# facebook/zstd

Hardware: NVIDIA H100
Metric: compress GB/s (input) at level 1 (higher is better)
Workload: dtype u8

## Files before the change

zstd_b200/csrc/zb_entropy.cuh:

```cuda
#ifndef ZB_ENTROPY_CUH
#define ZB_ENTROPY_CUH
#include "zb_device.cuh"

#define ZBD_ERR 0xFFFFFFFFu

struct ZbdBitW { u8* out; u32 pos; u64 acc; u32 nacc; };
__device__ __forceinline__ void zbd_bw_init(ZbdBitW* w, u8* out) { w->out = out; w->pos = 0; w->acc = 0; w->nacc = 0; }
__device__ __forceinline__ void zbd_bw_add(ZbdBitW* w, u32 value, u32 nbBits)
{
    if (!nbBits) return;
    w->acc |= (u64)(value & ((1u << nbBits) - 1u)) << w->nacc;
    w->nacc += nbBits;
    while (w->nacc >= 8) { w->out[w->pos++] = (u8)w->acc; w->acc >>= 8; w->nacc -= 8; }
}
__device__ __forceinline__ u32 zbd_bw_close(ZbdBitW* w)
{
    zbd_bw_add(w, 1, 1);
    if (w->nacc) w->out[w->pos++] = (u8)w->acc;
    return w->pos;
}


__device__ __forceinline__ u32 zbd_fse_optimalTableLog(u32 maxTableLog, u32 srcSize, u32 maxSymbolValue, u32 minus)
{
    u32 const fromSource = zb_hb32(srcSize - 1u) - minus;
    u32 const needSrc = zb_hb32(srcSize) + 1u, needAlphabet = zb_hb32(maxSymbolValue) + 2u;
    u32 const floorLog = needSrc < needAlphabet ? needSrc : needAlphabet;
    u32 log = maxTableLog < fromSource ? maxTableLog : fromSource;
    if (log < floorLog) log = floorLog;
    return log < 5u ? 5u : (log > 12u ? 12u : log);
}

__device__ inline u32 zbw_fse_normalize(short* norm, u32 tableLog, const u32* count, u32 total, u32 maxSymbolValue, u32 lane)
{
    u32 const T = 1u << tableLog;
    u32 base[2], rem[2]; bool present[2];
#pragma unroll
// ... 128 lines not shown
            u32 const owner = ls >> 1;
            u32 const before = __shfl_sync(ZB_FULL, (ls & 1u) ? seen1 : seen0, (int)owner);
            if (s == ls) ct->nextState[cum[ls] + before + (u32)__popc(grp & ((1u << lane) - 1u))] = (u16)(T + u);
            if (lane == owner) { if (ls & 1u) seen1 += (u32)__popc(grp); else seen0 += (u32)__popc(grp); }
            pending &= ~grp;
        }
    }
    __syncwarp();
}

__device__ inline void zbd_fse_buildCTable_rle(ZbdFseCTable* ct, u32 symbol)
{
    ct->tableLog = 0; ct->maxSymbolValue = symbol;
    ct->nextState[0] = 0; ct->nextState[1] = 0;
    ct->deltaNbBits[symbol] = 0; ct->deltaFindState[symbol] = 0;
}

__device__ __forceinline__ u32 zbd_fse_initState2(const ZbdFseCTable* ct, u32 symbol)
{
    u32 const dnb = ct->deltaNbBits[symbol];
    u32 const nbBitsOut = (dnb + (1u << 15)) >> 16;
    u32 const value = (nbBitsOut << 16) - dnb;
    return ct->nextState[(int)(value >> nbBitsOut) + ct->deltaFindState[symbol]];
}
__device__ __forceinline__ u32 zbd_fse_step(const ZbdFseCTable* ct, u32 state, u32 symbol, u32* bits, u32* nb)
{
    u32 const nbBitsOut = (state + ct->deltaNbBits[symbol]) >> 16;
    *nb = nbBitsOut;
    *bits = state & ((1u << nbBitsOut) - 1u);
    return ct->nextState[(int)(state >> nbBitsOut) + ct->deltaFindState[symbol]];
}

struct ZbdHufWksp {
    u32 A[256];
    u16 rankSym[256];
    u8  len[256];
    u8  weights[256];
    u32 nl[16];
    u32 firstCode[16];
    u32 wcount[16];
    short wnorm[16];
    u8  symAt[64];
    u16 cum[66];
    u32 maxLen, nz;
    ZbdFseCTable wct;
};

template <int HUF_THREADS>
__device__ inline u32 zbc_huf_build(ZbdHufWksp* w, const u32* count, u32 maxSymbolValue, u32 target, u32* enc)
{
    u32 const tid = threadIdx.x;
    if (tid == 0) w->nz = 0;
    __syncthreads();
    {   u32 mine = 0;
        for (u32 s = tid; s < 256u; s += HUF_THREADS) {
            u32 const c = s <= maxSymbolValue ? count[s] : 0u;
            w->len[s] = 0;
            if (c) {
                u32 r = 0;
                for (u32 j = 0; j <= maxSymbolValue; j++) { u32 const cj = count[j]; r += (cj > c || (cj == c && j < s)) ? 1u : 0u; }
                w->rankSym[r] = (u16)s;
                mine++;
            }
        }
        if (mine) atomicAdd(&w->nz, mine);
    }
    __syncthreads();
    u32 const nz = w->nz;
    for (u32 i = tid; i < nz; i += HUF_THREADS) w->A[i] = count[w->rankSym[nz - 1u - i]];
    __syncthreads();
    if (tid == 0) {
        u32* const A = w->A;
        u32 root = 0, leaf = 2, next;
        A[0] += A[1];
        for (next = 1; next + 1u < nz; next++) {
            if (leaf >= nz || A[root] < A[leaf]) { A[next] = A[root]; A[root++] = next; } else A[next] = A[leaf++];
            if (leaf >= nz || (root < next && A[root] < A[leaf])) { A[next] += A[root]; A[root++] = next; } else A[next] += A[leaf++];
        }
        A[nz - 2u] = 0;
        for (next = nz - 2u; next-- > 0u; ) A[next] = A[A[next]] + 1u;
        {   int avbl = 1, used = 0, depth = 0;
            int rt = (int)nz - 2, nx = (int)nz - 1;
            while (avbl > 0) {
                while (rt >= 0 && (int)A[rt] == depth) { used++; rt--; }
                while (avbl > used) { A[nx--] = (u32)depth; avbl--; }
                avbl = 2 * used; depth++; used = 0;
            }
        }
        for (u32 l = 0; l < 16u; l++) w->nl[l] = 0;
    }
    __syncthreads();
    u32 const deepest = w->A[0];
    for (u32 i = tid; i < nz; i += HUF_THREADS) { u32 const l = w->A[i]; atomicAdd(&w->nl[l < 15u ? l : 15u], 1u); }
    __syncthreads();
    if (tid == 0) {
        u32* const nl = w->nl;
        u32 maxLen = deepest;
        if (maxLen > target) {
            u32 K = 0;
            for (u32 l = target + 1u; l < 16u; l++) { nl[target] += nl[l]; nl[l] = 0; }
            for (u32 l = 1; l <= target; l++) K += nl[l] << (target - l);
            for (u32 E = K - (1u << target); E > 0u; E--) {
                u32 b = target - 1u;
                while (nl[b] == 0u) b--;
                nl[b]--; nl[b + 1u] += 2u; nl[target]--;
            }
            maxLen = target;
        }
        while (nl[maxLen] == 0u) maxLen--;
        w->maxLen = maxLen;
        u32 v = 0;
        for (u32 l = maxLen; l > 0u; l--) { w->firstCode[l] = v; v = (v + nl[l]) >> 1; }
    }
    __syncthreads();
    u32 const maxLen = w->maxLen;
    for (u32 r = tid; r < nz; r += HUF_THREADS) {
        u32 l = 1, acc = w->nl[1];
        while (r >= acc) { l++; acc += w->nl[l]; }
        w->len[w->rankSym[r]] = (u8)l;
    }
    __syncthreads();
    for (u32 s = tid; s < 256u; s += HUF_THREADS) {
        u32 const l = w->len[s];
        u32 e = 0;
        if (l) {
            u32 idx = 0;
            for (u32 j = 0; j < s; j++) idx += (w->len[j] == l) ? 1u : 0u;
            e = (w->firstCode[l] + idx) | (l << 16);
        }
        enc[s] = e;
    }
    __syncthreads();
    return maxLen;
}

template <int HUF_THREADS>
__device__ inline u32 zbc_huf_writeHeader(ZbdHufWksp* w, u8* dst, const u32* enc, u32 maxSymbolValue, u32 huffLog, u32* sh_result)
{
    u32 const tid = threadIdx.x, lane = tid & 31u;
    u8* const wt = w->weights;
    u32 const wtSize = maxSymbolValue;
    if (tid < 16u) w->wcount[tid] = 0;
    __syncthreads();
    for (u32 n = tid; n < wtSize; n += HUF_THREADS) {
        u32 const nb = enc[n] >> 16;
        u32 const v = nb ? huffLog + 1u - nb : 0u;
        wt[n] = (u8)v;
        atomicAdd(&w->wcount[v], 1u);
    }
    if (tid == 0) wt[wtSize] = 0;
    __syncthreads();
    if (tid < 32u) {
        u32 hSize = 0;
        if (wtSize > 2u) {
            u32 const c = lane < 13u ? w->wcount[lane] : 0u;
            u32 const used = __ballot_sync(ZB_FULL, c != 0u);
            u32 const maxSym = 31u - (u32)__clz((int)used);
            u32 maxCount = c;
#pragma unroll
            for (u32 o = 16; o > 0; o >>= 1) maxCount = max(maxCount, __shfl_xor_sync(ZB_FULL, maxCount, o));
            if (maxCount != wtSize && maxCount != 1u) {
                u32 const tableLog = zbd_fse_optimalTableLog(6, wtSize, maxSym, 2);
                u32 ok = zbw_fse_normalize(w->wnorm, tableLog, w->wcount, wtSize, maxSym, lane);
                u32 nc = 0;
                if (ok != ZBD_ERR) {
                    if (lane == 0) nc = zbd_fse_writeNCount(dst + 1, w->wnorm, maxSym, tableLog);
                    nc = __shfl_sync(ZB_FULL, nc, 0);
                    if (nc == ZBD_ERR) ok = ZBD_ERR;
                }
                if (ok != ZBD_ERR) {
                    zbw_fse_buildCTable(&w->wct, w->wnorm, maxSym, tableLog, w->symAt, w->cum, lane);
                    if (lane == 0) {
                        ZbdBitW bw; zbd_bw_init(&bw, dst + 1 + nc);
                        const u8* ip = wt + wtSize;
                        u32 s1, s2, bits, nb;
                        if (wtSize & 1u) {
                            s1 = zbd_fse_initState2(&w->wct, *--ip);
                            s2 = zbd_fse_initState2(&w->wct, *--ip);
                            s1 = zbd_fse_step(&w->wct, s1, *--ip, &bits, &nb); zbd_bw_add(&bw, bits, nb);
                        } else {
                            s2 = zbd_fse_initState2(&w->wct, *--ip);
                            s1 = zbd_fse_initState2(&w->wct, *--ip);
                        }
                        while (ip > wt) {
                            s2 = zbd_fse_step(&w->wct, s2, *--ip, &bits, &nb); zbd_bw_add(&bw, bits, nb);
                            s1 = zbd_fse_step(&w->wct, s1, *--ip, &bits, &nb); zbd_bw_add(&bw, bits, nb);
                        }
                        zbd_bw_add(&bw, s2, tableLog);
                        zbd_bw_add(&bw, s1, tableLog);
                        hSize = nc + zbd_bw_close(&bw);
                    }
                } else if (lane == 0) hSize = ZBD_ERR;
            } else if (maxCount == wtSize) hSize = 1;
        }
        if (lane == 0) {
            u32 res;
            if (hSize == ZBD_ERR) res = ZBD_ERR;
            else if (hSize > 1u && hSize < maxSymbolValue / 2u) { dst[0] = (u8)hSize; res = hSize + 1u; }
            else if (maxSymbolValue > 128u) res = ZBD_ERR;
            else {
                dst[0] = (u8)(128u + (maxSymbolValue - 1u));
                for (u32 n = 0; n < maxSymbolValue; n += 2u) dst[(n / 2u) + 1u] = (u8)((wt[n] << 4) + wt[n + 1u]);
                res = ((maxSymbolValue + 1u) / 2u) + 1u;
            }
            *sh_result = res;
        }
    }
    __syncthreads();
    return *sh_result;
}
#endif
```

zstd_b200/csrc/zb_literals.cu:

```cuda
#include "zb_entropy.cuh"
#include "zb_kernels.h"

#define LIT_THREADS 128
#ifndef LIT_MIN_CTAS
#define LIT_MIN_CTAS 12
#endif
#define LIT_WARPS (LIT_THREADS / 32)
#define LIT_WIN 256u

__device__ void zb_hist256(const u8* __restrict__ src, u32 n, u32 (*whist)[256], u32* count)
{
    u32 const tid = threadIdx.x, warp = tid >> 5, lane = tid & 31u;
    for (u32 i = tid; i < LIT_WARPS * 256; i += LIT_THREADS) (&whist[0][0])[i] = 0;
    __syncthreads();
    u32 const head = (u32)((uintptr_t)src & 15u);
    const uint4* const v4 = reinterpret_cast<const uint4*>(src - head);
    u32 const seg = (n + 3u) / 4u;
    u32 const beg = min(warp * seg, n) + head, end = min((warp + 1u) * seg, n) + head;
    if (beg < end) {
        u32 const vLo = beg >> 4, nVec = ((end - 1u) >> 4) - vLo + 1u;
        uint4 nx = lane < nVec ? __ldg(v4 + vLo + lane) : make_uint4(0, 0, 0, 0);
        for (u32 i = lane; i < nVec; i += 32u) {
            uint4 const q = nx;
            if (i + 32u < nVec) nx = __ldg(v4 + vLo + i + 32u);
            u32 const p0 = (vLo + i) << 4;
            u32 const kLo = beg > p0 ? beg - p0 : 0u, kHi = min(end - p0, 16u);
            u32 const w[4] = { q.x, q.y, q.z, q.w };
#pragma unroll
            for (u32 k = 0; k < 16u; k++)
                if (k >= kLo && k < kHi) atomicAdd(&whist[warp][(w[k >> 2] >> (8u * (k & 3u))) & 0xFFu], 1u);
        }
    }
    __syncthreads();
    for (u32 sym = tid; sym < 256u; sym += LIT_THREADS) {
        u32 s = 0;
#pragma unroll
        for (int w = 0; w < LIT_WARPS; w++) s += whist[w][sym];
        count[sym] = s;
    }
    __syncthreads();
}

__device__ void zb_hist_stats(const u32* count, u32* red, u32* largestOut, u32* maxSymOut)
{
    u32 const tid = threadIdx.x;
    u32 c = 0, key = 0;
    for (u32 sym = tid; sym < 256u; sym += LIT_THREADS) { u32 const v = count[sym]; c = max(c, v); key = max(key, v ? sym : 0u); }
#pragma unroll
    for (int o = 16; o > 0; o >>= 1) {
        c = max(c, __shfl_xor_sync(ZB_FULL, c, o));
        key = max(key, __shfl_xor_sync(ZB_FULL, key, o));
    }
    if ((tid & 31) == 0) { red[tid >> 5] = c; red[8 + (tid >> 5)] = key; }
    __syncthreads();
    if (tid == 0) {
        u32 l = 0, m = 0;
        for (int w = 0; w < LIT_WARPS; w++) { l = max(l, red[w]); m = max(m, red[8 + w]); }
        *largestOut = l; *maxSymOut = m;
    }
    __syncthreads();
}

__device__ __forceinline__ void zb_huf_stream(const u8* __restrict__ lit, u32 beg, u32 end, const u32* enc, u32* win, u32* ow,
                                              u32 bitPos, u32 lane)
{
    const uint4* const v4 = reinterpret_cast<const uint4*>(lit);
    uint4 const zero = make_uint4(0, 0, 0, 0);
    u32 const vHi = (end - 1u) >> 4, nVec = vHi - (beg >> 4) + 1u;
    u32 const firstW = bitPos >> 5;
    uint4 q1 = lane < nVec ? __ldg(v4 + vHi - lane) : zero;
    uint4 q2 = lane + 32u < nVec ? __ldg(v4 + vHi - lane - 32u) : zero;
    for (u32 t = 0; t < nVec; t += 32u) {
        uint4 const q = q1;
        q1 = q2;
        q2 = t + 64u + lane < nVec ? __ldg(v4 + vHi - (t + 64u + lane)) : zero;
        u32 kLo = 0, kHi = 0;
        if (t + lane < nVec) { u32 const p0 = (vHi - t - lane) << 4; kLo = beg > p0 ? beg - p0 : 0u; kHi = min(end - p0, 16u); }
        u32 const w[4] = { q.x, q.y, q.z, q.w };
        u32 nb = 0;
#pragma unroll
        for (u32 k = 0; k < 16u; k++) {
            u32 const e = enc[(w[k >> 2] >> (8u * (k & 3u))) & 0xFFu];
            nb += (k >= kLo && k < kHi) ? e >> 16 : 0u;
        }
        u32 incl = nb;
#pragma unroll
        for (u32 o = 1; o < 32u; o <<= 1) { u32 const x = __shfl_up_sync(ZB_FULL, incl, o); if (lane >= o) incl += x; }
        u32 const tileBits = __shfl_sync(ZB_FULL, incl, 31);
        {
            u32 const p = bitPos + incl - nb;
            u32 widx = p >> 5, nacc = p & 31u, first = 1;
            u64 acc = 0;
#pragma unroll
            for (int k = 15; k >= 0; k--) {
                u32 const e = ((u32)k >= kLo && (u32)k < kHi) ? enc[(w[k >> 2] >> (8u * (k & 3u))) & 0xFFu] : 0u;
                acc |= (u64)(e & 0xFFFFu) << nacc;
                nacc += e >> 16;
                if (k & 1) continue;
                bool const full = nacc >= 32u;
                u32* const wp = win + widx % LIT_WIN;
                if (full && first == 0u) *wp = (u32)acc;
                if (full && first != 0u) atomicOr(wp, (u32)acc);
                first = full ? 0u : first;
                widx += full ? 1u : 0u;
                acc = full ? (acc >> 32) : acc;
                nacc -= full ? 32u : 0u;
            }
            if (nacc != 0u && (u32)acc != 0u) atomicOr(win + widx % LIT_WIN, (u32)acc);
        }
        __syncwarp();
        u32 const wEnd = (bitPos + tileBits) >> 5;
        for (u32 k = (bitPos >> 5) + lane; k < wEnd; k += 32u) {
            u32 const v = win[k % LIT_WIN];
            win[k % LIT_WIN] = 0u;
            if (k == firstW) atomicOr(ow + k, v); else ow[k] = v;
        }
        __syncwarp();
        bitPos += tileBits;
    }
    if (lane == 0) atomicOr(ow + (bitPos >> 5), win[(bitPos >> 5) % LIT_WIN] | (1u << (bitPos & 31u)));
}

__global__ void __launch_bounds__(LIT_THREADS, LIT_MIN_CTAS)
zb_literals_kernel(const ZbBlock* __restrict__ blocks, ZbParams prm, ZbStrides sd, const ZbDictEntropy* __restrict__ deAll,
                   const ZbDictSlot* __restrict__ dicts, const u8* __restrict__ lits, u8* __restrict__ body, ZbBlockMeta* __restrict__ meta)
{
    __shared__ __align__(16) u32 whist[LIT_WARPS][256];
    __shared__ ZbdHufWksp wk;
    __shared__ u32 count[256];
    __shared__ u32 enc[256];
    __shared__ __align__(16) u8 hdr[288];
    __shared__ u32 red[16];
    __shared__ u32 sh_largest, sh_maxSym, sh_mode, sh_hSize, sh_usePrev;
    __shared__ u32 sh_bits[LIT_WARPS];

    u32 const tid = threadIdx.x, warp = tid >> 5, lane = tid & 31u;
    u32 const b = blockIdx.x;
    ZbBlockMeta const m = meta[b];
    if (m.forceRaw) return;
    u32 const n = m.litSize;
    const u8* const lit = lits + (size_t)b * sd.lit;
    u8* const out = body + (size_t)b * sd.body;
    enum { MODE_RAW = 0, MODE_RLE = 1, MODE_HUF = 2 };

    ZbBlock const bd = blocks[b];
    const ZbDictEntropy* const de = (bd.flags & ZB_FLAG_FIRST) ? (dicts ? dicts[bd.dictSlot].de : deAll) : nullptr;
    u32 repeat = (de != nullptr && de->present) ? de->hufRepeat : 0u;
    bool const preferRepeat = (n <= 1024u);
    u32 const lhSize = 3u + (n >= 1024u) + (n >= 16384u);
    u32 const nbStreams = (n < 256u || (repeat == 2u && lhSize == 3u)) ? 1u : 4u;
    u32 mode = MODE_HUF;
    bool usePrev = false;
    if (prm.litDisabled || n < (repeat == 2u ? 6u : 64u)) mode = MODE_RAW;
    if (mode == MODE_HUF && preferRepeat && repeat == 2u) usePrev = true;
    if (mode == MODE_HUF && !usePrev) {
        bool const suspect = (m.nbSeq == 0) || (n / m.nbSeq >= 20u);
        if (suspect && n >= 4096u * 10u) {
            u32 l1, l2;
            zb_hist256(lit, 4096u, whist, count);
            zb_hist_stats(count, red, &sh_largest, &sh_maxSym);
            l1 = sh_largest;
            __syncthreads();
            zb_hist256(lit + n - 4096u, 4096u, whist, count);
            zb_hist_stats(count, red, &sh_largest, &sh_maxSym);
            l2 = sh_largest;
            __syncthreads();
            if (l1 + l2 <= ((2u * 4096u) >> 7) + 4u) mode = MODE_RAW;
        }
    }
    if (mode == MODE_HUF) zb_hist256(lit, n, whist, count);
    if (mode == MODE_HUF && !usePrev) {
        zb_hist_stats(count, red, &sh_largest, &sh_maxSym);
        u32 const largest = sh_largest;
        if (largest == n) mode = MODE_RLE;
        else if (largest <= (n >> 7) + 4u) mode = MODE_RAW;
    }
    if (mode == MODE_HUF && !usePrev && repeat == 1u) {
        int bad = 0;
        for (u32 sym = tid; sym < 256u; sym += LIT_THREADS) bad |= (sym <= sh_maxSym) && count[sym] != 0u && (de->hufEnc[sym] >> 16) == 0u;
        if (__syncthreads_or(bad) || de->hufMaxSymbol < sh_maxSym) repeat = 0u;
    }
    if (mode == MODE_HUF && !usePrev && preferRepeat && repeat != 0u) usePrev = true;
    if (mode == MODE_HUF && !usePrev) {
        u32 const maxSym = sh_maxSym;
        u32 const huffLog = zbd_fse_optimalTableLog(11, n, maxSym, 1);
        u32 const maxBits = zbc_huf_build<LIT_THREADS>(&wk, count, maxSym, huffLog, enc);
        u32 const hSizeNew = (maxBits == ZBD_ERR) ? ZBD_ERR : zbc_huf_writeHeader<LIT_THREADS>(&wk, hdr, enc, maxSym, maxBits, &sh_hSize);
        if (tid == 0) {
            u32 md = MODE_HUF, hSize = 0, prev = 0;
            if (hSizeNew == ZBD_ERR) md = MODE_RAW;
            else {
                hSize = hSizeNew;
                if (repeat != 0u) {
                    u32 oldBits = 0, newBits = 0;
                    for (u32 sy = 0; sy <= maxSym; sy++) { oldBits += (de->hufEnc[sy] >> 16) * count[sy]; newBits += (enc[sy] >> 16) * count[sy]; }
                    if ((oldBits >> 3) <= hSize + (newBits >> 3) || hSize + 12u >= n) prev = 1;
                }
                if (!prev && hSize + 12u >= n) md = MODE_RAW;
            }
            sh_mode = md; sh_hSize = hSize; sh_usePrev = prev;
        }
        __syncthreads();
        mode = sh_mode;
        usePrev = sh_usePrev != 0u;
    }
    if (mode == MODE_HUF && usePrev) {
        __syncthreads();
        for (u32 sym = tid; sym < 256u; sym += LIT_THREADS) enc[sym] = de->hufEnc[sym];
        if (tid == 0) sh_hSize = 0;
        __syncthreads();
    }

    u32 const hType = usePrev ? 3u : 2u;
    u32 const seg = (n + 3u) / 4u;
    u32 streamSize[4] = { 0u, 0u, 0u, 0u };
    u32 hSize = 0, total = 0;
    if (mode == MODE_HUF) {
        hSize = sh_hSize;
        u32 bits = 0;
        for (u32 sym = lane; sym < 256u; sym += 32u) bits += whist[warp][sym] * (enc[sym] >> 16);
#pragma unroll
        for (int o = 16; o > 0; o >>= 1) bits += __shfl_xor_sync(ZB_FULL, bits, o);
        if (lane == 0) sh_bits[warp] = bits;
        __syncthreads();
        if (nbStreams == 4u) for (u32 k = 0; k < 4u; k++) streamSize[k] = (sh_bits[k] + 1u + 7u) >> 3;
        else streamSize[0] = (sh_bits[0] + sh_bits[1] + sh_bits[2] + sh_bits[3] + 1u + 7u) >> 3;
        u32 cSize = 0; bool tooBig = false;
#pragma unroll
        for (u32 k = 0; k < 4u; k++) { cSize += streamSize[k]; tooBig |= (streamSize[k] > 65535u); }
        if (nbStreams == 4u) cSize += 6u;
        total = hSize + cSize;
        if (nbStreams == 4u && tooBig) mode = MODE_RAW;
        else if (total >= n - 1u) mode = MODE_RAW;
        else if (total >= n - ((n >> 6) + 2u)) mode = MODE_RAW;
        else if (total == 1u) {
            int diff = 0;
            if (n < 8u) for (u32 i = tid; i < n; i += LIT_THREADS) diff |= (lit[i] != lit[0]);
            if (!__syncthreads_or(diff)) mode = MODE_RLE;
        }
    }

    if (mode == MODE_RAW) {
        u32 const flSize = 1u + (n > 31u) + (n > 4095u);
        if (tid == 0) {
            if (flSize == 1) out[0] = (u8)(0u + (n << 3));
            else if (flSize == 2) { u32 const v = 0u + (1u << 2) + (n << 4); out[0] = (u8)v; out[1] = (u8)(v >> 8); }
            else { u32 const v = 0u + (3u << 2) + (n << 4); out[0] = (u8)v; out[1] = (u8)(v >> 8); out[2] = (u8)(v >> 16); }
            meta[b].litSecSize = flSize + n;
        }
        for (u32 i = tid; i < n; i += LIT_THREADS) out[flSize + i] = lit[i];
        return;
    }
    if (mode == MODE_RLE) {
        if (tid == 0) {
            u32 const flSize = 1u + (n > 31u) + (n > 4095u);
            if (flSize == 1) out[0] = (u8)(1u + (n << 3));
            else if (flSize == 2) { u32 const v = 1u + (1u << 2) + (n << 4); out[0] = (u8)v; out[1] = (u8)(v >> 8); }
            else { u32 const v = 1u + (3u << 2) + (n << 4); out[0] = (u8)v; out[1] = (u8)(v >> 8); out[2] = (u8)(v >> 16); }
            out[flSize] = lit[0];
            meta[b].litSecSize = flSize + 1u;
        }
        return;
    }

    u32 sOff = lhSize + hSize + (nbStreams == 4u ? 6u : 0u), sSize = 0;
#pragma unroll
    for (u32 k = 0; k < 4u; k++) { sOff += k < warp ? streamSize[k] : 0u; sSize = k == warp ? streamSize[k] : sSize; }
    u32* const ow = reinterpret_cast<u32*>(out);
    for (u32 i = tid; i < LIT_WARPS * 256u; i += LIT_THREADS) (&whist[0][0])[i] = 0u;
    if (warp < nbStreams && lane == 0) { ow[sOff >> 2] = 0u; ow[(sOff + sSize - 1u) >> 2] = 0u; }
    __syncthreads();
    if (tid == 0) {
        u32 const cLitSize = total;
        if (lhSize == 3) { u32 const lhc = hType + ((nbStreams == 4u ? 1u : 0u) << 2) + (n << 4) + (cLitSize << 14);
                           out[0] = (u8)lhc; out[1] = (u8)(lhc >> 8); out[2] = (u8)(lhc >> 16); }
        else if (lhSize == 4) { u32 const lhc = hType + (2u << 2) + (n << 4) + (cLitSize << 18);
                           out[0] = (u8)lhc; out[1] = (u8)(lhc >> 8); out[2] = (u8)(lhc >> 16); out[3] = (u8)(lhc >> 24); }
        else { u32 const lhc = hType + (3u << 2) + (n << 4) + (cLitSize << 22);
                           out[0] = (u8)lhc; out[1] = (u8)(lhc >> 8); out[2] = (u8)(lhc >> 16); out[3] = (u8)(lhc >> 24);
                           out[4] = (u8)(cLitSize >> 10); }
        if (nbStreams == 4u) {
            u8* jt = out + lhSize + hSize;
            for (int k = 0; k < 3; k++) { jt[2 * k] = (u8)streamSize[k]; jt[2 * k + 1] = (u8)(streamSize[k] >> 8); }
        }
        meta[b].litSecSize = lhSize + total;
    }
    for (u32 i = tid; i < hSize; i += LIT_THREADS) out[lhSize + i] = hdr[i];
    __syncthreads();
    if (warp < nbStreams) {
        u32 const beg = nbStreams == 1u ? 0u : min(warp * seg, n), end = nbStreams == 1u ? n : min((warp + 1u) * seg, n);
        zb_huf_stream(lit, beg, end, enc, whist[warp], ow, sOff * 8u, lane);
    }
}

extern "C" cudaError_t zb_launch_literals(const ZbBlock* d_blocks, u32 nbBlocks, const ZbParams* prm, const ZbStrides* sd, const ZbDictEntropy* d_de,
                                          const u8* d_lits, u8* d_body, ZbBlockMeta* d_meta, cudaStream_t stream, const ZbDictSlot* d_dicts)
{
    if (nbBlocks == 0) return cudaSuccess;
    zb_literals_kernel<<<nbBlocks, LIT_THREADS, 0, stream>>>(d_blocks, *prm, *sd, d_de, d_dicts, d_lits, d_body, d_meta);
    return cudaGetLastError();
}
```

zstd_b200/csrc/zb_sequences.cu:

```cuda
#include "zb_entropy.cuh"
#include "zb_kernels.h"
#include "zb_bitpack.cuh"

#define SEQ_THREADS 128
#ifndef SEQ_TILE
#define SEQ_TILE 512u
#endif
#define MaxLL 35
#define MaxML 52
#define MaxOff 31
#define DefaultMaxOff 28
#define LLFSELog 9
#define MLFSELog 9
#define OffFSELog 8

__constant__ short c_LL_defaultNorm[MaxLL + 1] = { 4,3,2,2,2,2,2,2, 2,2,2,2,2,1,1,1, 2,2,2,2,2,2,2,2, 2,3,2,1,1,1,1,1, -1,-1,-1,-1 };
__constant__ short c_ML_defaultNorm[MaxML + 1] = { 1,4,3,2,2,2,2,2, 2,1,1,1,1,1,1,1, 1,1,1,1,1,1,1,1, 1,1,1,1,1,1,1,1,
                                                   1,1,1,1,1,1,1,1, 1,1,1,1,1,1,-1,-1, -1,-1,-1,-1,-1 };
__constant__ short c_OF_defaultNorm[DefaultMaxOff + 1] = { 1,1,1,1,1,1,2,2, 2,1,1,1,1,1,1,1, 1,1,1,1,1,1,1,1, -1,-1,-1,-1,-1 };

__device__ __forceinline__ u32 zbd_ll_code(u32 ll)
{
    if (ll > 63u) return zb_hb32(ll) + 19u;
    if (ll < 16u) return ll;
    if (ll < 24u) return 16u + ((ll - 16u) >> 1);
    if (ll < 32u) return 20u + ((ll - 24u) >> 2);
    if (ll < 48u) return 22u + ((ll - 32u) >> 3);
    return 24u;
}
__device__ __forceinline__ u32 zbd_ml_code(u32 mlBase)
{
    if (mlBase > 127u) return zb_hb32(mlBase) + 36u;
    if (mlBase < 32u) return mlBase;
    if (mlBase < 40u) return 32u + ((mlBase - 32u) >> 1);
    if (mlBase < 48u) return 36u + ((mlBase - 40u) >> 2);
    if (mlBase < 64u) return 38u + ((mlBase - 48u) >> 3);
    if (mlBase < 96u) return 40u + ((mlBase - 64u) >> 4);
    return 42u;
}
__device__ __forceinline__ u32 zbd_ll_lut_entry(u32 ll)
{
    u32 const c = zbd_ll_code(ll);
    return c | ((c < 16u ? 0u : (c < 20u ? 1u : (c < 22u ? 2u : (c < 24u ? 3u : 4u)))) << 8);
}
__device__ __forceinline__ u32 zbd_ml_lut_entry(u32 mlBase)
{
    u32 const c = zbd_ml_code(mlBase);
    return c | ((c < 32u ? 0u : (c < 36u ? 1u : (c < 38u ? 2u : (c < 40u ? 3u : (c < 42u ? 4u : 5u))))) << 8);
// ... 35 lines not shown
    return cudaMemcpyToSymbolAsync(g_defaultCT, host3, 3 * sizeof(ZbdFseCTable), 0, cudaMemcpyHostToDevice, stream);
}

struct ZbdStreamWork {
    u32 count[64];
    short norm[64];
    u8  nc[136];
    u8  symAt[512];
    u16 cum[66];
    u32 ncSize;
    u32 type;
    u32 finalState;
    u32 err;
};

__global__ void __launch_bounds__(SEQ_THREADS)
zb_sequences_kernel(const u8* __restrict__ src, const ZbBlock* __restrict__ blocks, ZbParams prm, ZbStrides sd, const ZbDictEntropy* __restrict__ deAll,
                    const ZbDictSlot* __restrict__ dicts,
                    const u64* __restrict__ seqs, u16* __restrict__ stateBits,
                    u8* __restrict__ body, ZbBlockMeta* __restrict__ meta)
{
    __shared__ ZbdFseCTable ct[3];
    __shared__ ZbdStreamWork wk[3];
    __shared__ u32 chunkBits[SEQ_THREADS];
    __shared__ u32 stepTile[3][SEQ_TILE + 3u];
    __shared__ u32 sh_cSize, sh_hdrEnd, sh_streamSize;
    __shared__ ZbdCodeLut lut;

    u32 const tid = threadIdx.x;
    u32 const b = blockIdx.x;
    ZbBlockMeta const m = meta[b];
    ZbBlock const bd = blocks[b];
    if (m.forceRaw) return;
    const ZbDictEntropy* const de = (bd.flags & ZB_FLAG_FIRST) ? (dicts ? dicts[bd.dictSlot].de : deAll) : nullptr;
    u32 const nbSeq = m.nbSeq;
    const u64* const myseq = seqs + (size_t)b * sd.seq;
    u16* const myst = stateBits + (size_t)b * sd.dist;
    u8* const out = body + (size_t)b * sd.body;
    u32 op = m.litSecSize;

    u32 const nbSeqHdr = nbSeq < 128u ? 1u : (nbSeq < 0x7F00u ? 2u : 3u);
    if (tid == 0) {
        if (nbSeq < 128u) out[op] = (u8)nbSeq;
        else if (nbSeq < 0x7F00u) { out[op] = (u8)((nbSeq >> 8) + 0x80u); out[op + 1] = (u8)nbSeq; }
        else { out[op] = 0xFF; out[op + 1] = (u8)(nbSeq - 0x7F00u); out[op + 2] = (u8)((nbSeq - 0x7F00u) >> 8); }
    }
    op += nbSeqHdr;
    u32 cSize;
    if (nbSeq == 0) {
        cSize = op;
    } else {
        for (u32 i = tid; i < 192u; i += SEQ_THREADS) wk[i >> 6].count[i & 63u] = 0;
        for (u32 i = tid; i < 192u; i += SEQ_THREADS) { if (i < 64u) lut.ll[i] = (u16)zbd_ll_lut_entry(i); else lut.ml[i - 64u] = (u16)zbd_ml_lut_entry(i - 64u); }
        __syncthreads();
        for (u32 i = tid; i < nbSeq; i += SEQ_THREADS) {
            ZbdSeq const s = zbd_unpack(myseq[i], lut);
            atomicAdd(&wk[0].count[s.llc], 1u);
            atomicAdd(&wk[1].count[s.ofc], 1u);
            atomicAdd(&wk[2].count[s.mlc], 1u);
        }
        __syncthreads();
        if (tid < 96u) {
            u32 const st = tid >> 5, lane = tid & 31u;
            ZbdStreamWork* const w = &wk[st];
            u32 const maxAll = st == 0 ? MaxLL : (st == 1 ? MaxOff : MaxML);
            u32 const c0 = w->count[lane], c1 = (lane + 32u <= maxAll) ? w->count[lane + 32u] : 0u;
            u32 const hiUsed = __ballot_sync(ZB_FULL, c1 != 0u), loUsed = __ballot_sync(ZB_FULL, c0 != 0u);
            u32 const max = hiUsed ? 63u - (u32)__clz((int)hiUsed) : 31u - (u32)__clz((int)loUsed);
            u32 mostFrequent = c0 > c1 ? c0 : c1;
#pragma unroll
            for (u32 o = 16; o > 0; o >>= 1) mostFrequent = ::max(mostFrequent, __shfl_xor_sync(ZB_FULL, mostFrequent, o));
            u32 const defLog = st == 1 ? 5u : 6u;
            bool const defAllowed = st == 1 ? (max <= DefaultMaxOff) : true;
            u32 const prevRepeat = (de != nullptr && de->present) ? de->fseRepeat[st] : 0u;
            u32 const type = zbd_selectEncodingType(mostFrequent, nbSeq, defLog, defAllowed, prm.strategy, prevRepeat);
            if (lane == 0) { w->type = type; w->err = 0; w->ncSize = 0; }
            __syncwarp();
            if (type == set_repeat || type == set_basic) {
                const u32* from = reinterpret_cast<const u32*>(type == set_repeat ? &de->fse[st] : &g_defaultCT[st]);
                u32* to = reinterpret_cast<u32*>(&ct[st]);
                for (u32 i = lane; i < sizeof(ZbdFseCTable) / 4u; i += 32u) to[i] = from[i];
            } else if (type == set_rle) {
                if (lane == 0) {
                    ZbdSeq const first = zbd_unpack(myseq[0], lut);
                    u32 const sym = st == 0 ? first.llc : (st == 1 ? first.ofc : first.mlc);
                    zbd_fse_buildCTable_rle(&ct[st], max);
                    w->nc[0] = (u8)sym; w->ncSize = 1;
                }
            } else {
                u32 const FSELog = st == 1 ? OffFSELog : (st == 0 ? LLFSELog : MLFSELog);
                u32 nbSeq_1 = nbSeq;
                u32 const tableLog = zbd_fse_optimalTableLog(FSELog, nbSeq, max, 2);
                {
                    ZbdSeq const last = zbd_unpack(myseq[nbSeq - 1], lut);
                    u32 const lastCode = st == 0 ? last.llc : (st == 1 ? last.ofc : last.mlc);
                    if (w->count[lastCode] > 1u) { nbSeq_1--; __syncwarp(); if (lane == 0) w->count[lastCode]--; }
                    __syncwarp();
                }
                u32 const r = zbw_fse_normalize(w->norm, tableLog, w->count, nbSeq_1, max, lane);
                u32 ncs = 0;
                if (r != ZBD_ERR) { if (lane == 0) ncs = zbd_fse_writeNCount(w->nc, w->norm, max, tableLog); ncs = __shfl_sync(ZB_FULL, ncs, 0); }
                if (r == ZBD_ERR || ncs == ZBD_ERR) { if (lane == 0) w->err = 1; }
                else {
                    if (lane == 0) w->ncSize = ncs;
                    zbw_fse_buildCTable(&ct[st], w->norm, max, tableLog, w->symAt, w->cum, lane);
                }
            }
        }
        __syncthreads();
        bool const err = wk[0].err | wk[1].err | wk[2].err;
        if (err) { if (tid == 0) { meta[b].type = ZB_BT_RAW; meta[b].bodySize = bd.size; } return; }

        {
            u32 state = 0;
            bool const chain = tid < 3u;
            u32 const st = chain ? tid : 0u;
            const u16* const ns = ct[st].nextState;
            const u32* const tw = stepTile[st] + 1;
            u16* const rec = myst + (size_t)st * sd.state;
            u32 const nbTiles = (nbSeq + SEQ_TILE - 1u) / SEQ_TILE;
            for (u32 tile = nbTiles; tile-- > 0; ) {
                u32 const t0 = tile * SEQ_TILE, t1 = min(t0 + SEQ_TILE, nbSeq);
                for (u32 i = t0 + tid; i < t1; i += SEQ_THREADS) {
                    ZbdSeq const s = zbd_unpack(myseq[i], lut);
                    stepTile[0][i - t0 + 1u] = ct[0].deltaNbBits[s.llc] | ((u32)ct[0].deltaFindState[s.llc] << 20);
                    stepTile[1][i - t0 + 1u] = ct[1].deltaNbBits[s.ofc] | ((u32)ct[1].deltaFindState[s.ofc] << 20);
                    stepTile[2][i - t0 + 1u] = ct[2].deltaNbBits[s.mlc] | ((u32)ct[2].deltaFindState[s.mlc] << 20);
                }
                __syncthreads();
                if (chain) {
                    u32 cnt = t1 - t0;
                    const u32* pw = tw + cnt;
                    u16* pr = rec + t1;
                    if (t1 == nbSeq) {
                        u32 const w0 = pw[-1], dnb = w0 & 0xFFFFFu;
                        u32 const nbOut = (dnb + (1u << 15)) >> 16;
                        state = ns[(int)(((nbOut << 16) - dnb) >> nbOut) + ((int)w0 >> 20)];
                        cnt--; pw--; pr--;
                    }
                    u32 w = pw[-1];
                    while (cnt) {
                        cnt--; pw--; pr--;
                        u32 const wn = pw[-1];
                        u32 const nb = (state + (w & 0xFFFFFu)) >> 16;
                        *pr = (u16)((state & ((1u << nb) - 1u)) | (nb << 12));
                        state = ns[(int)(state >> nb) + ((int)w >> 20)];
                        w = wn;
                    }
                }
                __syncthreads();
            }
            if (chain) wk[st].finalState = state;
        }
        __syncthreads();

        u32 const ncTotal = wk[0].ncSize + wk[1].ncSize + wk[2].ncSize;
        u32 const hdrEnd = op + 1u + ncTotal;
        u32 lastCountSize = 0;
        if (wk[0].type == set_compressed) lastCountSize = wk[0].ncSize;
        if (wk[1].type == set_compressed) lastCountSize = wk[1].ncSize;
        if (wk[2].type == set_compressed) lastCountSize = wk[2].ncSize;

        u32 const cs = (nbSeq + SEQ_THREADS - 1u) / SEQ_THREADS;
        u32 const cBeg = min(tid * cs, nbSeq), cEnd = min((tid + 1u) * cs, nbSeq);
        u32 bits = 0;
        for (u32 i = cBeg; i < cEnd; i++) {
            ZbdSeq const s = zbd_unpack(myseq[i], lut);
            bits += s.llBits + s.mlBits + s.ofc;
            if (i + 1u < nbSeq) bits += (myst[i] >> 12) + (myst[sd.state + i] >> 12) + (myst[2u * sd.state + i] >> 12);
        }
        chunkBits[tid] = bits;
        __syncthreads();
        u32 bitOff = 0;
        for (u32 k = tid + 1u; k < SEQ_THREADS; k++) bitOff += chunkBits[k];
        if (tid == 0) {
            u32 const totalBits = bitOff + bits + ct[2].tableLog + ct[1].tableLog + ct[0].tableLog + 1u;
            sh_streamSize = (totalBits + 7u) >> 3;
        }
        __syncthreads();
        u32 const streamSize = sh_streamSize;
        cSize = hdrEnd + streamSize;
        bool const fits = (cSize + 16u <= sd.body);
        if (fits) {
            u32 const w0 = hdrEnd >> 2, w1 = (cSize + 3u) >> 2;
            u32* const ow = reinterpret_cast<u32*>(out);
            for (u32 i = w0 + 1u + tid; i < w1; i += SEQ_THREADS) ow[i] = 0;
            if (tid == 0) {
                for (u32 i = hdrEnd; i < min((w0 + 1u) << 2, cSize + 4u); i++) out[i] = 0;
                u8* p = out + op;
                *p++ = (u8)((wk[0].type << 6) + (wk[1].type << 4) + (wk[2].type << 2));
                for (u32 st = 0; st < 3; st++) for (u32 i = 0; i < wk[st].ncSize; i++) *p++ = wk[st].nc[i];
            }
            __syncthreads();
            ZbdParW pw; zbd_pw_init(&pw, ow, (u64)hdrEnd * 8u + bitOff);
            for (u32 i = cEnd; i-- > cBeg; ) {
                ZbdSeq const s = zbd_unpack(myseq[i], lut);
                if (i + 1u < nbSeq) {
                    u32 const rOF = myst[sd.state + i], rML = myst[2u * sd.state + i], rLL = myst[i];
                    zbd_pw_add(&pw, rOF & 0xFFFu, rOF >> 12);
                    zbd_pw_add(&pw, rML & 0xFFFu, rML >> 12);
                    zbd_pw_add(&pw, rLL & 0xFFFu, rLL >> 12);
                }
                u32 const llb = s.llBits, mlb = s.mlBits;
                zbd_pw_add(&pw, s.litLen & ((1u << llb) - 1u), llb);
                zbd_pw_add(&pw, s.mlBase & ((1u << mlb) - 1u), mlb);
                zbd_pw_add(&pw, s.offBase & ((1u << s.ofc) - 1u), s.ofc);
            }
            if (tid == 0) {
                zbd_pw_add(&pw, wk[2].finalState & ((1u << ct[2].tableLog) - 1u), ct[2].tableLog);
                zbd_pw_add(&pw, wk[1].finalState & ((1u << ct[1].tableLog) - 1u), ct[1].tableLog);
                zbd_pw_add(&pw, wk[0].finalState & ((1u << ct[0].tableLog) - 1u), ct[0].tableLog);
                zbd_pw_add(&pw, 1u, 1u);
            }
            zbd_pw_finish(&pw);
        }
        if (!fits || (lastCountSize && (lastCountSize + streamSize) < 4u)) cSize = 0;
    }

    {   u32 const maxCSize = bd.size - ((bd.size >> 6) + 2u);
        if (cSize >= maxCSize) cSize = 0;
    }
    bool rle = false;
    if (!(bd.flags & ZB_FLAG_FIRST) && cSize < 25u) {
        const u8* const bsrc = src + bd.srcOff;
        u8 const v0 = bsrc[0];
        int diff = 0;
        for (u32 i = tid; i < bd.size; i += SEQ_THREADS) diff |= (bsrc[i] != v0);
        rle = !__syncthreads_or(diff);
    }
    if (tid == 0) {
        ZbBlockMeta mm = m;
        if (rle) { mm.type = ZB_BT_RLE; mm.bodySize = 1; mm.rleByte = src[bd.srcOff]; }
        else if (cSize == 0) { mm.type = ZB_BT_RAW; mm.bodySize = bd.size; }
        else { mm.type = ZB_BT_COMPRESSED; mm.bodySize = cSize; }
        meta[b] = mm;
    }
}

extern "C" cudaError_t zb_launch_sequences(const u8* d_src, const ZbBlock* d_blocks, u32 nbBlocks, const ZbParams* prm, const ZbStrides* sd, const ZbDictEntropy* d_de,
                                           const u64* d_seqs, u16* d_stateBits, u8* d_body, ZbBlockMeta* d_meta, cudaStream_t stream,
                                           const ZbDictSlot* d_dicts)
{
    if (nbBlocks == 0) return cudaSuccess;
    zb_sequences_kernel<<<nbBlocks, SEQ_THREADS, 0, stream>>>(d_src, d_blocks, *prm, *sd, d_de, d_dicts, d_seqs, d_stateBits, d_body, d_meta);
    return cudaGetLastError();
}
```

Measured before the change: 108.9.

## Parallelize Huffman build, header FSE encode, and literal stream packing

Symbol ranking in the Huffman build now uses packed count/symbol keys compared four at a time with vector loads, and the symbol count comes from __syncthreads_count. Code assignment per length uses warp match_any plus per-chunk prefix counts instead of an O(n^2) scan. The weight-header FSE encode splits into two lanes for state stepping, then a warp-wide scan and atomicOr bit packing. The literal histogram gains a fast path for full vectors, and Huffman stream encoding caches packed codes in shared memory instead of looking enc up twice. Optional clock instrumentation is added behind a compile flag. The shared histogram buffer doubles in size, which may lower occupancy.

After: 110.6 (median of 6 runs). 1.6% higher.

```diff
diff --git a/zstd_b200/csrc/zb_entropy.cuh b/zstd_b200/csrc/zb_entropy.cuh
--- a/zstd_b200/csrc/zb_entropy.cuh
+++ b/zstd_b200/csrc/zb_entropy.cuh
@@ -3,6 +3,27 @@
 #include "zb_device.cuh"
 
 #define ZBD_ERR 0xFFFFFFFFu
+
+#define ZB_CLK_SLOTS 16
+#ifdef ZB_ENTROPY_CLOCKS
+struct ZbClockRows { unsigned long long* rows; u32 cap; u32 next; };
+static __shared__ unsigned long long* zb_clkRow;
+__device__ __forceinline__ void zb_clk_begin(ZbClockRows* r)
+{
+    if (threadIdx.x == 0) {
+        u32 const i = atomicAdd(&r->next, 1u);
+        zb_clkRow = i < r->cap ? r->rows + (size_t)i * ZB_CLK_SLOTS : nullptr;
+        if (zb_clkRow) { u32 sm; asm volatile("mov.u32 %0, %%smid;" : "=r"(sm)); zb_clkRow[14] = sm; zb_clkRow[0] = clock64(); }
+    }
+}
+#define ZB_CLK(k) do { if (threadIdx.x == 0 && zb_clkRow) zb_clkRow[k] = clock64(); } while (0)
+#define ZB_CLK_TAG(v) do { if (threadIdx.x == 0 && zb_clkRow) zb_clkRow[13] = (v); } while (0)
+#define ZB_CLK_SYNC() __syncthreads()
+#else
+#define ZB_CLK(k) ((void)0)
+#define ZB_CLK_TAG(v) ((void)0)
+#define ZB_CLK_SYNC() ((void)0)
+#endif
 
 struct ZbdBitW { u8* out; u32 pos; u64 acc; u32 nacc; };
 __device__ __forceinline__ void zbd_bw_init(ZbdBitW* w, u8* out) { w->out = out; w->pos = 0; w->acc = 0; w->nacc = 0; }
@@ -197,7 +218,7 @@
 }
 
 struct ZbdHufWksp {
-    u32 A[256];
+    __align__(16) u32 A[256];
     u16 rankSym[256];
     u8  len[256];
     u8  weights[256];
@@ -207,33 +228,35 @@
     short wnorm[16];
     u8  symAt[64];
     u16 cum[66];
-    u32 maxLen, nz;
+    u32 maxLen;
     ZbdFseCTable wct;
 };
 
 template <int HUF_THREADS>
 __device__ inline u32 zbc_huf_build(ZbdHufWksp* w, const u32* count, u32 maxSymbolValue, u32 target, u32* enc)
 {
-    u32 const tid = threadIdx.x;
-    if (tid == 0) w->nz = 0;
-    __syncthreads();
-    {   u32 mine = 0;
-        for (u32 s = tid; s < 256u; s += HUF_THREADS) {
-            u32 const c = s <= maxSymbolValue ? count[s] : 0u;
-            w->len[s] = 0;
-            if (c) {
-                u32 r = 0;
-                for (u32 j = 0; j <= maxSymbolValue; j++) { u32 const cj = count[j]; r += (cj > c || (cj == c && j < s)) ? 1u : 0u; }
-                w->rankSym[r] = (u16)s;
-                mine++;
-            }
-        }
-        if (mine) atomicAdd(&w->nz, mine);
-    }
-    __syncthreads();
-    u32 const nz = w->nz;
+    static_assert(HUF_THREADS == 128, "two symbols per thread");
+    u32 const tid = threadIdx.x, lane = tid & 31u;
+    u32 const s0 = tid, s1 = tid + 128u;
+    u32 const k0 = s0 <= maxSymbolValue && count[s0] ? (count[s0] << 8) | (255u - s0) : 0u;
+    u32 const k1 = s1 <= maxSymbolValue && count[s1] ? (count[s1] << 8) | (255u - s1) : 0u;
+    w->A[s0] = k0; w->A[s1] = k1;
+    w->len[s0] = 0; w->len[s1] = 0;
+    __syncthreads();
+    {   u32 r0 = 0, r1 = 0;
+        const uint4* const k4 = reinterpret_cast<const uint4*>(w->A);
+        for (u32 v = 0; v <= (maxSymbolValue >> 2); v++) {
+            uint4 const q = k4[v];
+            r0 += (q.x > k0) + (q.y > k0) + (q.z > k0) + (q.w > k0);
+            r1 += (q.x > k1) + (q.y > k1) + (q.z > k1) + (q.w > k1);
+        }
+        if (k0) w->rankSym[r0] = (u16)s0;
+        if (k1) w->rankSym[r1] = (u16)s1;
+    }
+    u32 const nz = (u32)__syncthreads_count(k0 != 0u) + (u32)__syncthreads_count(k1 != 0u);
     for (u32 i = tid; i < nz; i += HUF_THREADS) w->A[i] = count[w->rankSym[nz - 1u - i]];
     __syncthreads();
+    ZB_CLK(3);
     if (tid == 0) {
         u32* const A = w->A;
         u32 root = 0, leaf = 2, next;
@@ -255,6 +278,7 @@
         for (u32 l = 0; l < 16u; l++) w->nl[l] = 0;
     }
     __syncthreads();
+    ZB_CLK(4);
     u32 const deepest = w->A[0];
     for (u32 i = tid; i < nz; i += HUF_THREADS) { u32 const l = w->A[i]; atomicAdd(&w->nl[l < 15u ? l : 15u], 1u); }
     __syncthreads();
@@ -284,18 +308,26 @@
         while (r >= acc) { l++; acc += w->nl[l]; }
         w->len[w->rankSym[r]] = (u8)l;
     }
-    __syncthreads();
+    u32* const chunkLen = w->A;
+    chunkLen[tid] = 0;
+    __syncthreads();
+    ZB_CLK(5);
+    u32 const below = (1u << lane) - 1u;
+#pragma unroll
     for (u32 s = tid; s < 256u; s += HUF_THREADS) {
-        u32 const l = w->len[s];
-        u32 e = 0;
-        if (l) {
-            u32 idx = 0;
-            for (u32 j = 0; j < s; j++) idx += (w->len[j] == l) ? 1u : 0u;
-            e = (w->firstCode[l] + idx) | (l << 16);
-        }
-        enc[s] = e;
-    }
-    __syncthreads();
+        u32 const l = w->len[s], g = __match_any_sync(ZB_FULL, l);
+        if ((g & below) == 0u) chunkLen[(s >> 5) * 16u + l] = (u32)__popc(g);
+    }
+    __syncthreads();
+#pragma unroll
+    for (u32 s = tid; s < 256u; s += HUF_THREADS) {
+        u32 const l = w->len[s], g = __match_any_sync(ZB_FULL, l);
+        u32 idx = (u32)__popc(g & below);
+        for (u32 c = 0; c < (s >> 5); c++) idx += chunkLen[c * 16u + l];
+        enc[s] = l ? (w->firstCode[l] + idx) | (l << 12) | (l << 16) : 0u;
+    }
+    __syncthreads();
+    ZB_CLK(6);
     return maxLen;
 }
 
@@ -335,26 +367,52 @@
                 }
                 if (ok != ZBD_ERR) {
                     zbw_fse_buildCTable(&w->wct, w->wnorm, maxSym, tableLog, w->symAt, w->cum, lane);
+                    u32* const rec = w->A;
+                    u32 st = 0;
+                    if (lane < 2u) {
+                        u32 i = ((wtSize - 1u) & 1u) == lane ? wtSize - 1u : wtSize - 2u;
+                        st = zbd_fse_initState2(&w->wct, wt[i]);
+                        while (i >= 2u) {
+                            u32 bits, nb;
+                            i -= 2u;
+                            st = zbd_fse_step(&w->wct, st, wt[i], &bits, &nb);
+                            rec[i] = bits | (nb << 16);
+                        }
+                    }
+                    u32 const sEven = __shfl_sync(ZB_FULL, st, 0), sOdd = __shfl_sync(ZB_FULL, st, 1);
+                    u32 const nE = wtSize - 2u, per = (nE + 31u) >> 5;
+                    u32 const e0 = min(lane * per, nE), e1 = min(e0 + per, nE);
+                    u32 mine = 0;
+                    for (u32 e = e0; e < e1; e++) mine += rec[wtSize - 3u - e] >> 16;
+                    u32 incl = mine;
+#pragma unroll
+                    for (u32 o = 1; o < 32u; o <<= 1) { u32 const x = __shfl_up_sync(ZB_FULL, incl, o); if (lane >= o) incl += x; }
+                    u32 const fieldBits = __shfl_sync(ZB_FULL, incl, 31);
+                    u32 const sBytes = (fieldBits + 2u * tableLog + 1u + 7u) >> 3;
+                    u8* const sp = dst + 1 + nc;
+                    for (u32 k = lane; k < sBytes; k += 32u) sp[k] = 0;
+                    __syncwarp();
+                    u32 const mis = (u32)((uintptr_t)sp & 3u);
+                    u32* const wb = reinterpret_cast<u32*>(sp - mis);
+                    {   u32 const p = mis * 8u + incl - mine;
+                        u32 widx = p >> 5, nacc = p & 31u;
+                        u64 acc = 0;
+                        for (u32 e = e0; e < e1; e++) {
+                            u32 const r = rec[wtSize - 3u - e];
+                            acc |= (u64)(r & 0xFFFFu) << nacc;
+                            nacc += r >> 16;
+                            if (nacc >= 32u) { atomicOr(wb + widx, (u32)acc); acc >>= 32; nacc -= 32u; widx++; }
+                        }
+                        if ((u32)acc) atomicOr(wb + widx, (u32)acc);
+                    }
                     if (lane == 0) {
-                        ZbdBitW bw; zbd_bw_init(&bw, dst + 1 + nc);
-                        const u8* ip = wt + wtSize;
-                        u32 s1, s2, bits, nb;
-                        if (wtSize & 1u) {
-                            s1 = zbd_fse_initState2(&w->wct, *--ip);
-                            s2 = zbd_fse_initState2(&w->wct, *--ip);
-                            s1 = zbd_fse_step(&w->wct, s1, *--ip, &bits, &nb); zbd_bw_add(&bw, bits, nb);
-                        } else {
-                            s2 = zbd_fse_initState2(&w->wct, *--ip);
-                            s1 = zbd_fse_initState2(&w->wct, *--ip);
-                        }
-                        while (ip > wt) {
-                            s2 = zbd_fse_step(&w->wct, s2, *--ip, &bits, &nb); zbd_bw_add(&bw, bits, nb);
-                            s1 = zbd_fse_step(&w->wct, s1, *--ip, &bits, &nb); zbd_bw_add(&bw, bits, nb);
-                        }
-                        zbd_bw_add(&bw, s2, tableLog);
-                        zbd_bw_add(&bw, s1, tableLog);
-                        hSize = nc + zbd_bw_close(&bw);
+                        u32 const m = (1u << tableLog) - 1u, p = mis * 8u + fieldBits, o = p & 31u;
+                        u32 const v = (sOdd & m) | ((sEven & m) << tableLog) | (1u << (2u * tableLog));
+                        atomicOr(wb + (p >> 5), v << o);
+                        if (o + 2u * tableLog + 1u > 32u) atomicOr(wb + (p >> 5) + 1u, v >> (32u - o));
                     }
+                    __syncwarp();
+                    hSize = nc + sBytes;
                 } else if (lane == 0) hSize = ZBD_ERR;
             } else if (maxCount == wtSize) hSize = 1;
         }
diff --git a/zstd_b200/csrc/zb_literals.cu b/zstd_b200/csrc/zb_literals.cu
--- a/zstd_b200/csrc/zb_literals.cu
+++ b/zstd_b200/csrc/zb_literals.cu
@@ -8,11 +8,21 @@
 #define LIT_WARPS (LIT_THREADS / 32)
 #define LIT_WIN 256u
 
-__device__ void zb_hist256(const u8* __restrict__ src, u32 n, u32 (*whist)[256], u32* count)
+#ifdef ZB_ENTROPY_CLOCKS
+__device__ ZbClockRows g_litClocks;
+extern "C" __attribute__((visibility("default"))) cudaError_t zb_literals_clocks(unsigned long long* rows, u32 cap)
+{
+    ZbClockRows const r = { rows, cap, 0u };
+    return cudaMemcpyToSymbol(g_litClocks, &r, sizeof(r));
+}
+#endif
+
+__device__ void zb_hist256(const u8* __restrict__ src, u32 n, u32 (*whist)[512], u32* count)
 {
     u32 const tid = threadIdx.x, warp = tid >> 5, lane = tid & 31u;
-    for (u32 i = tid; i < LIT_WARPS * 256; i += LIT_THREADS) (&whist[0][0])[i] = 0;
-    __syncthreads();
+    for (u32 i = tid; i < LIT_WARPS * 256; i += LIT_THREADS) whist[i >> 8][i & 255u] = 0;
+    __syncthreads();
+    u32* const bins = whist[warp];
     u32 const head = (u32)((uintptr_t)src & 15u);
     const uint4* const v4 = reinterpret_cast<const uint4*>(src - head);
     u32 const seg = (n + 3u) / 4u;
@@ -26,9 +36,14 @@
             u32 const p0 = (vLo + i) << 4;
             u32 const kLo = beg > p0 ? beg - p0 : 0u, kHi = min(end - p0, 16u);
             u32 const w[4] = { q.x, q.y, q.z, q.w };
-#pragma unroll
-            for (u32 k = 0; k < 16u; k++)
-                if (k >= kLo && k < kHi) atomicAdd(&whist[warp][(w[k >> 2] >> (8u * (k & 3u))) & 0xFFu], 1u);
+            if (kLo == 0u && kHi == 16u) {
+#pragma unroll
+                for (u32 k = 0; k < 16u; k++) atomicAdd(&bins[__byte_perm(w[k >> 2], 0u, 0x4440u | (k & 3u))], 1u);
+            } else {
+#pragma unroll
+                for (u32 k = 0; k < 16u; k++)
+                    if (k >= kLo && k < kHi) atomicAdd(&bins[__byte_perm(w[k >> 2], 0u, 0x4440u | (k & 3u))], 1u);
+            }
         }
     }
     __syncthreads();
@@ -64,6 +79,7 @@
 __device__ __forceinline__ void zb_huf_stream(const u8* __restrict__ lit, u32 beg, u32 end, const u32* enc, u32* win, u32* ow,
                                               u32 bitPos, u32 lane)
 {
+    uint4* const cache = reinterpret_cast<uint4*>(win + LIT_WIN);
     const uint4* const v4 = reinterpret_cast<const uint4*>(lit);
     uint4 const zero = make_uint4(0, 0, 0, 0);
     u32 const vHi = (end - 1u) >> 4, nVec = vHi - (beg >> 4) + 1u;
@@ -78,10 +94,17 @@
         if (t + lane < nVec) { u32 const p0 = (vHi - t - lane) << 4; kLo = beg > p0 ? beg - p0 : 0u; kHi = min(end - p0, 16u); }
         u32 const w[4] = { q.x, q.y, q.z, q.w };
         u32 nb = 0;
-#pragma unroll
-        for (u32 k = 0; k < 16u; k++) {
-            u32 const e = enc[(w[k >> 2] >> (8u * (k & 3u))) & 0xFFu];
-            nb += (k >= kLo && k < kHi) ? e >> 16 : 0u;
+        {
+            u32 pk[8];
+#pragma unroll
+            for (u32 k = 0; k < 16u; k += 2u) {
+                u32 const e0 = (k >= kLo && k < kHi) ? enc[(w[k >> 2] >> (8u * (k & 3u))) & 0xFFu] : 0u;
+                u32 const e1 = (k + 1u >= kLo && k + 1u < kHi) ? enc[(w[k >> 2] >> (8u * ((k + 1u) & 3u))) & 0xFFu] : 0u;
+                nb += (e0 >> 16) + (e1 >> 16);
+                pk[k >> 1] = __byte_perm(e0, e1, 0x5410);
+            }
+            cache[lane] = make_uint4(pk[0], pk[1], pk[2], pk[3]);
+            cache[32u + lane] = make_uint4(pk[4], pk[5], pk[6], pk[7]);
         }
         u32 incl = nb;
 #pragma unroll
@@ -91,11 +114,14 @@
             u32 const p = bitPos + incl - nb;
             u32 widx = p >> 5, nacc = p & 31u, first = 1;
             u64 acc = 0;
+            uint4 c = cache[32u + lane];
 #pragma unroll
             for (int k = 15; k >= 0; k--) {
-                u32 const e = ((u32)k >= kLo && (u32)k < kHi) ? enc[(w[k >> 2] >> (8u * (k & 3u))) & 0xFFu] : 0u;
-                acc |= (u64)(e & 0xFFFFu) << nacc;
-                nacc += e >> 16;
+                if (k == 7) c = cache[lane];
+                u32 const cw = (k & 4) ? ((k & 2) ? c.w : c.z) : ((k & 2) ? c.y : c.x);
+                u32 const e = (k & 1) ? cw >> 16 : cw & 0xFFFFu;
+                acc |= (u64)(e & 0xFFFu) << nacc;
+                nacc += e >> 12;
                 if (k & 1) continue;
                 bool const full = nacc >= 32u;
                 u32* const wp = win + widx % LIT_WIN;
@@ -125,7 +151,7 @@
 zb_literals_kernel(const ZbBlock* __restrict__ blocks, ZbParams prm, ZbStrides sd, const ZbDictEntropy* __restrict__ deAll,
                    const ZbDictSlot* __restrict__ dicts, const u8* __restrict__ lits, u8* __restrict__ body, ZbBlockMeta* __restrict__ meta)
 {
-    __shared__ __align__(16) u32 whist[LIT_WARPS][256];
+    __shared__ __align__(16) u32 whist[LIT_WARPS][512];
     __shared__ ZbdHufWksp wk;
     __shared__ u32 count[256];
     __shared__ u32 enc[256];
@@ -138,6 +164,9 @@
     u32 const b = blockIdx.x;
     ZbBlockMeta const m = meta[b];
     if (m.forceRaw) return;
+#ifdef ZB_ENTROPY_CLOCKS
+    zb_clk_begin(&g_litClocks);
+#endif
     u32 const n = m.litSize;
     const u8* const lit = lits + (size_t)b * sd.lit;
     u8* const out = body + (size_t)b * sd.body;
@@ -169,6 +198,7 @@
         }
     }
     if (mode == MODE_HUF) zb_hist256(lit, n, whist, count);
+    ZB_CLK(1);
     if (mode == MODE_HUF && !usePrev) {
         zb_hist_stats(count, red, &sh_largest, &sh_maxSym);
         u32 const largest = sh_largest;
@@ -181,11 +211,13 @@
         if (__syncthreads_or(bad) || de->hufMaxSymbol < sh_maxSym) repeat = 0u;
     }
     if (mode == MODE_HUF && !usePrev && preferRepeat && repeat != 0u) usePrev = true;
+    ZB_CLK_SYNC(); ZB_CLK(2);
     if (mode == MODE_HUF && !usePrev) {
         u32 const maxSym = sh_maxSym;
         u32 const huffLog = zbd_fse_optimalTableLog(11, n, maxSym, 1);
         u32 const maxBits = zbc_huf_build<LIT_THREADS>(&wk, count, maxSym, huffLog, enc);
         u32 const hSizeNew = (maxBits == ZBD_ERR) ? ZBD_ERR : zbc_huf_writeHeader<LIT_THREADS>(&wk, hdr, enc, maxSym, maxBits, &sh_hSize);
+        ZB_CLK(7);
         if (tid == 0) {
             u32 md = MODE_HUF, hSize = 0, prev = 0;
             if (hSizeNew == ZBD_ERR) md = MODE_RAW;
@@ -203,10 +235,11 @@
         __syncthreads();
         mode = sh_mode;
         usePrev = sh_usePrev != 0u;
+        ZB_CLK(8);
     }
     if (mode == MODE_HUF && usePrev) {
         __syncthreads();
-        for (u32 sym = tid; sym < 256u; sym += LIT_THREADS) enc[sym] = de->hufEnc[sym];
+        for (u32 sym = tid; sym < 256u; sym += LIT_THREADS) { u32 const h = de->hufEnc[sym]; enc[sym] = h | ((h >> 16) << 12); }
         if (tid == 0) sh_hSize = 0;
         __syncthreads();
     }
@@ -239,6 +272,8 @@
             if (!__syncthreads_or(diff)) mode = MODE_RLE;
         }
     }
+    ZB_CLK_SYNC(); ZB_CLK(9);
+    ZB_CLK_TAG(mode | (usePrev ? 4u : 0u) | (nbStreams << 4));
 
     if (mode == MODE_RAW) {
         u32 const flSize = 1u + (n > 31u) + (n > 4095u);
@@ -249,6 +284,7 @@
             meta[b].litSecSize = flSize + n;
         }
         for (u32 i = tid; i < n; i += LIT_THREADS) out[flSize + i] = lit[i];
+        ZB_CLK_SYNC(); ZB_CLK(15);
         return;
     }
     if (mode == MODE_RLE) {
@@ -260,6 +296,7 @@
             out[flSize] = lit[0];
             meta[b].litSecSize = flSize + 1u;
         }
+        ZB_CLK(15);
         return;
     }
 
@@ -267,7 +304,7 @@
 #pragma unroll
     for (u32 k = 0; k < 4u; k++) { sOff += k < warp ? streamSize[k] : 0u; sSize = k == warp ? streamSize[k] : sSize; }
     u32* const ow = reinterpret_cast<u32*>(out);
-    for (u32 i = tid; i < LIT_WARPS * 256u; i += LIT_THREADS) (&whist[0][0])[i] = 0u;
+    for (u32 i = tid; i < LIT_WARPS * LIT_WIN; i += LIT_THREADS) whist[i / LIT_WIN][i % LIT_WIN] = 0u;
     if (warp < nbStreams && lane == 0) { ow[sOff >> 2] = 0u; ow[(sOff + sSize - 1u) >> 2] = 0u; }
     __syncthreads();
     if (tid == 0) {
@@ -287,10 +324,12 @@
     }
     for (u32 i = tid; i < hSize; i += LIT_THREADS) out[lhSize + i] = hdr[i];
     __syncthreads();
+    ZB_CLK(10);
     if (warp < nbStreams) {
         u32 const beg = nbStreams == 1u ? 0u : min(warp * seg, n), end = nbStreams == 1u ? n : min((warp + 1u) * seg, n);
         zb_huf_stream(lit, beg, end, enc, whist[warp], ow, sOff * 8u, lane);
     }
+    ZB_CLK_SYNC(); ZB_CLK(11); ZB_CLK(15);
 }
 
 extern "C" cudaError_t zb_launch_literals(const ZbBlock* d_blocks, u32 nbBlocks, const ZbParams* prm, const ZbStrides* sd, const ZbDictEntropy* d_de,
diff --git a/zstd_b200/csrc/zb_sequences.cu b/zstd_b200/csrc/zb_sequences.cu
--- a/zstd_b200/csrc/zb_sequences.cu
+++ b/zstd_b200/csrc/zb_sequences.cu
@@ -14,6 +14,15 @@
 #define MLFSELog 9
 #define OffFSELog 8
 
+#ifdef ZB_ENTROPY_CLOCKS
+__device__ ZbClockRows g_seqClocks;
+extern "C" __attribute__((visibility("default"))) cudaError_t zb_sequences_clocks(unsigned long long* rows, u32 cap)
+{
+    ZbClockRows const r = { rows, cap, 0u };
+    return cudaMemcpyToSymbol(g_seqClocks, &r, sizeof(r));
+}
+#endif
+
 __constant__ short c_LL_defaultNorm[MaxLL + 1] = { 4,3,2,2,2,2,2,2, 2,2,2,2,2,1,1,1, 2,2,2,2,2,2,2,2, 2,3,2,1,1,1,1,1, -1,-1,-1,-1 };
 __constant__ short c_ML_defaultNorm[MaxML + 1] = { 1,4,3,2,2,2,2,2, 2,1,1,1,1,1,1,1, 1,1,1,1,1,1,1,1, 1,1,1,1,1,1,1,1,
                                                    1,1,1,1,1,1,1,1, 1,1,1,1,1,1,-1,-1, -1,-1,-1,-1,-1 };
@@ -115,6 +124,10 @@
     ZbBlockMeta const m = meta[b];
     ZbBlock const bd = blocks[b];
     if (m.forceRaw) return;
+#ifdef ZB_ENTROPY_CLOCKS
+    zb_clk_begin(&g_seqClocks);
+#endif
+    ZB_CLK_TAG(m.nbSeq);
     const ZbDictEntropy* const de = (bd.flags & ZB_FLAG_FIRST) ? (dicts ? dicts[bd.dictSlot].de : deAll) : nullptr;
     u32 const nbSeq = m.nbSeq;
     const u64* const myseq = seqs + (size_t)b * sd.seq;
@@ -143,6 +156,7 @@
             atomicAdd(&wk[2].count[s.mlc], 1u);
         }
         __syncthreads();
+        ZB_CLK(1);
         if (tid < 96u) {
             u32 const st = tid >> 5, lane = tid & 31u;
             ZbdStreamWork* const w = &wk[st];
@@ -181,16 +195,20 @@
                     __syncwarp();
                 }
                 u32 const r = zbw_fse_normalize(w->norm, tableLog, w->count, nbSeq_1, max, lane);
+                ZB_CLK(2);
                 u32 ncs = 0;
                 if (r != ZBD_ERR) { if (lane == 0) ncs = zbd_fse_writeNCount(w->nc, w->norm, max, tableLog); ncs = __shfl_sync(ZB_FULL, ncs, 0); }
+                ZB_CLK(3);
                 if (r == ZBD_ERR || ncs == ZBD_ERR) { if (lane == 0) w->err = 1; }
                 else {
                     if (lane == 0) w->ncSize = ncs;
                     zbw_fse_buildCTable(&ct[st], w->norm, max, tableLog, w->symAt, w->cum, lane);
-                }
-            }
-        }
-        __syncthreads();
+                    ZB_CLK(4);
+                }
+            }
+        }
+        __syncthreads();
+        ZB_CLK(5);
         bool const err = wk[0].err | wk[1].err | wk[2].err;
         if (err) { if (tid == 0) { meta[b].type = ZB_BT_RAW; meta[b].bodySize = bd.size; } return; }
 
@@ -236,6 +254,7 @@
             if (chain) wk[st].finalState = state;
         }
         __syncthreads();
+        ZB_CLK(6);
 
         u32 const ncTotal = wk[0].ncSize + wk[1].ncSize + wk[2].ncSize;
         u32 const hdrEnd = op + 1u + ncTotal;
@@ -262,6 +281,7 @@
         }
         __syncthreads();
         u32 const streamSize = sh_streamSize;
+        ZB_CLK(7);
         cSize = hdrEnd + streamSize;
         bool const fits = (cSize + 16u <= sd.body);
         if (fits) {
@@ -297,6 +317,7 @@
             }
             zbd_pw_finish(&pw);
         }
+        ZB_CLK_SYNC(); ZB_CLK(8);
         if (!fits || (lastCountSize && (lastCountSize + streamSize) < 4u)) cSize = 0;
     }
 
@@ -318,6 +339,7 @@
         else { mm.type = ZB_BT_COMPRESSED; mm.bodySize = cSize; }
         meta[b] = mm;
     }
+    ZB_CLK(15);
 }
 
 extern "C" cudaError_t zb_launch_sequences(const u8* d_src, const ZbBlock* d_blocks, u32 nbBlocks, const ZbParams* prm, const ZbStrides* sd, const ZbDictEntropy* d_de,
```
